# LukasHedegaard/continual-skeletons

Hardware: AMD Instinct MI355X
Metric: clips/sec (ST-GCN clip forward, NTU-60 shape; CoST-GCN online step reported under costgcn_online) (higher is better)
Workload: dtype f32

## Files before the change

### continual-skeletons_amd/csrc/gcn.hip

```cpp
#include <type_traits>

#include "mfma_core.h"
#include "gcn_params.h"


template <int MT, int NJ>
__global__ __launch_bounds__(NTHREADS, 2) void gcn_stage_kernel(const GcnParams p) {
    constexpr int NT = 16384 / MT;
    constexpr int WM = MT / 64;
    constexpr int TPC = NTHREADS / NT;
    constexpr int KPT = KC / TPC;
    extern __shared__ __attribute__((aligned(16))) float smem[];
    const int V = p.V, R = p.R, EW = p.ell_w;
    float *Wl = smem;
    float *Xa = Wl + R * KC * MT;
    float *Bx = Xa + R * KC * NT;
    float *Lv = Bx + KC * p.ldb;
    int *Ls = reinterpret_cast<int *>(Lv + 3 * V * EW * (p.adj_per_frame ? p.lds_frames : 1));

    const int tid = threadIdx.x, lane = tid & 63, wave = __builtin_amdgcn_readfirstlane(tid >> 6);
    const int wm = wave % WM, wn = wave / WM;
    const int l31 = lane & 31, kh = lane >> 5;
    const unsigned wid = xcd_contiguous_id(blockIdx.x, gridDim.x);
    const int m0 = (int)(wid % p.mtiles) * MT, q0 = (int)((wid / p.mtiles) % p.qtiles) * NT;
// ... 135 lines not shown
    } else {
#pragma unroll
        for (int mi = 0; mi < 2; ++mi)
#pragma unroll
            for (int g = 0; g < 16; ++g) bb[mi][g] = p.bias[rbase + mi * 32 + 4 * kh + (g & 3) + 8 * (g >> 2)];
#pragma unroll
        for (int ni = 0; ni < 2; ++ni) {
            const int qc = min(q0 + wn * 64 + ni * 32 + l31, Q - 1);
#pragma unroll
            for (int mi = 0; mi < 2; ++mi)
#pragma unroll
                for (int g = 0; g < 16; ++g) {
                    const int co = rbase + mi * 32 + 4 * kh + (g & 3) + 8 * (g >> 2);
                    rv[ni][mi][g] = ident ? seg_base[(int64_t)min(co, p.Cout - 1) * p.x_chan_stride + qc] : 0.f;
                }
        }
    }
#pragma unroll
    for (int mi = 0; mi < 2; ++mi)
#pragma unroll
        for (int g = 0; g < 16; ++g) {
            const float v0 = relu_nan(acc[mi][0][g] + bb[mi][g] + rv[0][mi][g]);
            const float v1 = relu_nan(acc[mi][1][g] + bb[mi][g] + rv[1][mi][g]);
            const auto sw = __builtin_amdgcn_permlane32_swap(__float_as_uint(v0), __float_as_uint(v1), false, false);
            acc[mi][0][g] = __uint_as_float(sw[0]);
            acc[mi][1][g] = __uint_as_float(sw[1]);
        }
    const int qb = q0 + wn * 64 + lane;
    const bool qv = qb < Q;
    if (full) {
        if (qv) {
            const unsigned qo = 4u * (unsigned)qb;
#pragma unroll
            for (int mi = 0; mi < 2; ++mi)
#pragma unroll
                for (int g = 0; g < 16; ++g) {
                    float *orow = oseg + (int64_t)(rbase + mi * 32 + (g & 3) + 8 * (g >> 2)) * p.y_chan_stride;
                    st_lane(orow, qo, acc[mi][0][g]);
                    st_lane(orow + 4 * p.y_chan_stride, qo, acc[mi][1][g]);
                }
        }
    } else {
#pragma unroll
        for (int mi = 0; mi < 2; ++mi)
#pragma unroll
            for (int g = 0; g < 16; ++g) {
                const int row0 = rbase + mi * 32 + (g & 3) + 8 * (g >> 2);
                if (qv && row0 < p.Cout) oseg[(int64_t)row0 * p.y_chan_stride + qb] = acc[mi][0][g];
                if (qv && row0 + 4 < p.Cout) oseg[(int64_t)(row0 + 4) * p.y_chan_stride + qb] = acc[mi][1][g];
            }
    }
}

template <int MT, bool CONVRES, int KCG_, bool PLAIN = false, bool SPLIT = false>
__global__ __launch_bounds__(NTHREADS, 3) void gcn_stage_sparse2_kernel(const GcnParams p) {
    constexpr int NT = 16384 / MT;
    constexpr int WM = MT / 64;
    constexpr int R = PLAIN ? 1 : (CONVRES ? 4 : 3);
    constexpr int M4 = MT / 4;
    constexpr int WB = (R * KCG_ * M4 + NTHREADS - 1) / NTHREADS;
    constexpr int RPW = KCG_ / (NTHREADS / 64);
    constexpr int NJ = MT == 128 ? 3 : 5;
    constexpr int NS = KCG_ / 2;
    constexpr int NH = NS / 2;
    static_assert(KCG_ % 8 == 0, "a chunk is a whole number of rows per wave");
    extern __shared__ __attribute__((aligned(16))) float smem[];
    const int V = p.V;
    const int wsz = R * KCG_ * MT, bsz = KCG_ * p.ldb, bufsz = wsz + bsz;

    const int tid = threadIdx.x, lane = tid & 63, wave = __builtin_amdgcn_readfirstlane(tid >> 6);
    const int wm = wave % WM, wn = wave / WM;
    const int l31 = lane & 31, kh = lane >> 5;
    const unsigned wid = xcd_contiguous_id(blockIdx.x, gridDim.x);
    const int m0 = (int)(wid % p.mtiles) * MT, q0 = (int)((wid / p.mtiles) % p.qtiles) * NT;
    const int segks = (int)(wid / (p.mtiles * p.qtiles));
    const int seg = SPLIT ? segks / p.ksplit : segks, ks = SPLIT ? segks % p.ksplit : 0;
    const int cb = SPLIT ? ks * p.cper : 0;
    const int Q = p.frames * V;
    const int qend = min(q0 + NT, Q);
    const int ta = div_magic(q0, p.vmagic), tb = div_magic(qend - 1, p.vmagic);
    const int span = (tb - ta + 1) * V;
    int eoff[2][6];
    float eval[2][6];
    int ioff[2];
#pragma unroll
    for (int ni = 0; ni < 2; ++ni) {
        const int q = min(q0 + wn * 64 + ni * 32 + l31, Q - 1);
        const int t = div_magic(q, p.vmagic);
        const int w = q - t * V, fb = (t - ta) * V;
        ioff[ni] = fb + w;
#pragma unroll
        for (int e = 0; e < 6; ++e) {
            const int r = e < 2 ? e : 2, k = e < 2 ? 0 : e - 2;
            const bool have = !PLAIN && k < p.ell_cnt[r];
            const int idx = PLAIN ? 0 : (r * V + w) * p.ell_w + min(k, p.ell_w - 1);
            eoff[ni][e] = fb + (have ? p.ell_src[idx] : 0);
            eval[ni][e] = have ? p.ell_val[idx] : 0.f;
        }
    }

    f32x16 acc[2][2];
#pragma unroll
    for (int a = 0; a < 2; ++a)
#pragma unroll
        for (int b = 0; b < 2; ++b)
#pragma unroll
            for (int g = 0; g < 16; ++g) acc[a][b][g] = 0.f;

    const float *seg_base = p.x + (int64_t)seg * p.x_seg_stride;
    const float *wbase = p.w + m0 + (size_t)cb * p.Mpad;
    f32x4 wv[WB];
    unsigned wgo[WB], wlo[WB];
#pragma unroll
    for (int u = 0; u < WB; ++u) {
        const int e = min(u * NTHREADS + tid, R * KCG_ * M4 - 1);
        const int row = e / M4, m4 = e % M4;
        wgo[u] = (unsigned)(((row / KCG_) * p.CinPad + (row % KCG_)) * p.Mpad + m4 * 4);
        wlo[u] = (unsigned)(e * 4);
    }
    constexpr int NJ4 = (NJ + 3) / 4;
    float bv[RPW][NJ];
    f32x4 bv4[RPW][NJ4];
    unsigned bgo[NJ], blo[NJ];
#pragma unroll
    for (int u = 0; u < NJ; ++u) {
        const int j = min(u * 64 + lane, span - 1);
        bgo[u] = (unsigned)(ta * V + j);
        blo[u] = (unsigned)j;
    }
    const int nvec = (span + 3) / 4;
    const bool vec = ta * V + 4 * nvec <= Q && p.Cin >= KCG_;
    unsigned bgo4[NJ4], blo4[NJ4];
#pragma unroll
    for (int u = 0; u < NJ4; ++u) {
        const int i = min(u * 64 + lane, nvec - 1);
        bgo4[u] = (unsigned)(ta * V + 4 * i);
        blo4[u] = (unsigned)(4 * i);
    }
    auto issue_one = [&](auto vtag, int i, int c0) {
        constexpr bool VEC = decltype(vtag)::value;
        constexpr int NX = VEC ? NJ4 : NJ;
        if (i < WB) {
            wv[i] = *reinterpret_cast<const f32x4 *>(wbase + (size_t)c0 * p.Mpad + wgo[i]);
        } else {
            const int rr = (i - WB) / NX, u = (i - WB) % NX;
            const int c = min(cb + c0 + wave + rr * (NTHREADS / 64), p.Cin - 1);
            const float *row = seg_base + (int64_t)c * p.x_chan_stride;
            if (VEC) bv4[rr][u] = *reinterpret_cast<const f32x4u *>(row + bgo4[u]);
            else bv[rr][u] = row[bgo[u]];
        }
    };
    auto commit = [&](auto vtag, float *buf) {
        constexpr bool VEC = decltype(vtag)::value;
        float *Wl = buf, *Bx = buf + wsz;
#pragma unroll
        for (int u = 0; u < WB; ++u) *reinterpret_cast<f32x4 *>(Wl + wlo[u]) = wv[u];
#pragma unroll
        for (int rr = 0; rr < RPW; ++rr) {
            float *dst = Bx + (wave + rr * (NTHREADS / 64)) * p.ldb;
            if (VEC) {
#pragma unroll
                for (int u = 0; u < NJ4; ++u) *reinterpret_cast<f32x4 *>(dst + blo4[u]) = bv4[rr][u];
            } else {
#pragma unroll
                for (int u = 0; u < NJ; ++u) dst[blo[u]] = bv[rr][u];
            }
        }
    };
    const int offA = wm * 64 + l31;
    auto mfma_step = [&](const float *buf, int s) {
        const float *Wl = buf, *Bx = buf + wsz;
        const int kk = 2 * s + kh;
        const float *bx = Bx + kk * p.ldb;
        float b[R][2];
#pragma unroll
        for (int ni = 0; ni < 2; ++ni) {
            if constexpr (PLAIN) {
                b[0][ni] = bx[ioff[ni]];
            } else {
                const float x0 = bx[eoff[ni][0]];
                b[0][ni] = eval[ni][0] * x0;
                b[1][ni] = eval[ni][1] * bx[eoff[ni][1]];
                float s2 = eval[ni][2] * bx[eoff[ni][2]];
                s2 = fmaf(eval[ni][3], bx[eoff[ni][3]], s2);
                s2 = fmaf(eval[ni][4], bx[eoff[ni][4]], s2);
                s2 = fmaf(eval[ni][5], bx[eoff[ni][5]], s2);
                b[2][ni] = s2;
                if (CONVRES) b[R - 1][ni] = bx[ioff[ni]];
            }
        }
#pragma unroll
        for (int r = 0; r < R; ++r) {
            const float *wr = Wl + (r * KCG_ + kk) * MT + offA;
            const float a0 = wr[0], a1 = wr[32];
            acc[0][0] = __builtin_amdgcn_mfma_f32_32x32x2f32(a0, b[r][0], acc[0][0], 0, 0, 0);
            acc[0][1] = __builtin_amdgcn_mfma_f32_32x32x2f32(a0, b[r][1], acc[0][1], 0, 0, 0);
            acc[1][0] = __builtin_amdgcn_mfma_f32_32x32x2f32(a1, b[r][0], acc[1][0], 0, 0, 0);
            acc[1][1] = __builtin_amdgcn_mfma_f32_32x32x2f32(a1, b[r][1], acc[1][1], 0, 0, 0);
        }
    };

    const int nchunks = (SPLIT ? min(p.CinPad - cb, p.cper) : p.CinPad) / KCG_;
    auto k_loop = [&](auto vtag) {
        constexpr int NLX = WB + RPW * (decltype(vtag)::value ? NJ4 : NJ);
#pragma unroll
        for (int i = 0; i < NLX; ++i) issue_one(vtag, i, 0);
        commit(vtag, smem);
        if (nchunks > 1) {
#pragma unroll
            for (int i = 0; i < NLX; ++i) issue_one(vtag, i, KCG_);
        }
        __syncthreads();
        for (int c = 0; c + 1 < nchunks; ++c) {
            float *cur = smem + (c & 1) * bufsz, *oth = smem + ((c & 1) ^ 1) * bufsz;
            commit(vtag, oth);
            const int cnext = min(c + 2, nchunks - 1) * KCG_;
            __builtin_amdgcn_s_setprio(1);
#pragma unroll
            for (int s = 0; s < NS; ++s) {
                if (s < NH) {
#pragma unroll
                    for (int i = s * NLX / NH; i < (s + 1) * NLX / NH; ++i) issue_one(vtag, i, cnext);
                    __builtin_amdgcn_sched_barrier(0);
                }
                mfma_step(cur, s);
            }
            __builtin_amdgcn_s_setprio(0);
            __syncthreads();
        }
    };
    if (vec) k_loop(std::true_type{});
    else k_loop(std::false_type{});
    const float *last = smem + ((nchunks - 1) & 1) * bufsz;
    const int rbase = m0 + wm * 64;
    const bool full = p.fast_epi && m0 + MT <= p.Cout;
    const unsigned kh4 = 4u * (unsigned)kh;
    float *oseg = SPLIT ? p.part + (int64_t)(seg * p.ksplit + ks) * p.Cout * p.y_chan_stride : p.y + (int64_t)seg * p.y_seg_stride;
    const int qb = q0 + wn * 64 + lane;
    const bool qv = qb < Q;
    float bb[2][16], rv[2][2][16];
    auto load_half = [&](int mi) {
        if (SPLIT) {
#pragma unroll
            for (int g = 0; g < 16; ++g) bb[mi][g] = rv[0][mi][g] = rv[1][mi][g] = 0.f;
        } else if (full) {
#pragma unroll
            for (int g = 0; g < 16; ++g) bb[mi][g] = ld_lane(p.bias + (rbase + mi * 32 + (g & 3) + 8 * (g >> 2)), kh4 * 4u);
#pragma unroll
            for (int ni = 0; ni < 2; ++ni) {
                const unsigned lo = 4u * (kh4 * (unsigned)p.x_chan_stride + (unsigned)min(q0 + wn * 64 + ni * 32 + l31, Q - 1));
#pragma unroll
                for (int g = 0; g < 16; ++g) {
                    const float *rrow = seg_base + (int64_t)(rbase + mi * 32 + (g & 3) + 8 * (g >> 2)) * p.x_chan_stride;
                    rv[ni][mi][g] = (CONVRES || PLAIN) ? 0.f : ld_lane(rrow, lo);
                }
            }
        } else {
#pragma unroll
            for (int g = 0; g < 16; ++g) bb[mi][g] = p.bias[rbase + mi * 32 + 4 * kh + (g & 3) + 8 * (g >> 2)];
#pragma unroll
            for (int ni = 0; ni < 2; ++ni) {
                const int qc = min(q0 + wn * 64 + ni * 32 + l31, Q - 1);
#pragma unroll
                for (int g = 0; g < 16; ++g) {
                    const int co = rbase + mi * 32 + 4 * kh + (g & 3) + 8 * (g >> 2);
                    rv[ni][mi][g] = (CONVRES || PLAIN) ? 0.f : seg_base[(int64_t)min(co, p.Cout - 1) * p.x_chan_stride + qc];
                }
            }
        }
    };
    auto finish_half = [&](int mi) {
#pragma unroll
        for (int g = 0; g < 16; ++g) {
            float v0 = acc[mi][0][g] + bb[mi][g] + rv[0][mi][g];
            float v1 = acc[mi][1][g] + bb[mi][g] + rv[1][mi][g];
            if (!PLAIN && !SPLIT) { v0 = relu_nan(v0); v1 = relu_nan(v1); }
            const auto sw = __builtin_amdgcn_permlane32_swap(__float_as_uint(v0), __float_as_uint(v1), false, false);
            acc[mi][0][g] = __uint_as_float(sw[0]);
            acc[mi][1][g] = __uint_as_float(sw[1]);
        }
        if (full) {
            if (qv) {
                const unsigned qo = 4u * (unsigned)qb;
#pragma unroll
                for (int g = 0; g < 16; ++g) {
                    float *orow = oseg + (int64_t)(rbase + mi * 32 + (g & 3) + 8 * (g >> 2)) * p.y_chan_stride;
                    st_lane(orow, qo, acc[mi][0][g]);
                    st_lane(orow + 4 * p.y_chan_stride, qo, acc[mi][1][g]);
                }
            }
        } else {
#pragma unroll
            for (int g = 0; g < 16; ++g) {
                const int row0 = rbase + mi * 32 + (g & 3) + 8 * (g >> 2);
                if (qv && row0 < p.Cout) oseg[(int64_t)row0 * p.y_chan_stride + qb] = acc[mi][0][g];
                if (qv && row0 + 4 < p.Cout) oseg[(int64_t)(row0 + 4) * p.y_chan_stride + qb] = acc[mi][1][g];
            }
        }
    };
#pragma unroll
    for (int s = 0; s < NS; ++s) mfma_step(last, s);
    load_half(0);
    finish_half(0);
    load_half(1);
    finish_half(1);
}

template <int MT, bool CONVRES, int KC2, int OCC>
__global__ __launch_bounds__(NTHREADS, OCC) void gcn_stage_dense_kernel(const GcnParams p) {
    constexpr int NT = 16384 / MT;
    constexpr int WM = MT / 64;
    constexpr int R = CONVRES ? 4 : 3;
    constexpr int M4 = MT / 4;
    constexpr int WB = R * KC2 * M4 / NTHREADS;
    constexpr int WBU = (R * KC2 * M4 + NTHREADS - 1) / NTHREADS;
    extern __shared__ __attribute__((aligned(16))) float smem[];
    const int V = p.V, FT = p.lds_frames, ldbx = p.ldb;
    float *Wl = smem;
    float *Xa = Wl + R * KC2 * MT;
    float *Bx = Xa + 3 * KC2 * NT;
    float *Ladj = Bx + KC2 * ldbx;

    const int tid = threadIdx.x, lane = tid & 63, wave = __builtin_amdgcn_readfirstlane(tid >> 6);
    const int wm = wave % WM, wn = wave / WM;
    const int l31 = lane & 31, kh = lane >> 5;
    const unsigned wid = xcd_contiguous_id(blockIdx.x, gridDim.x);
    const int m0 = (int)(wid % p.mtiles) * MT, qt = (int)((wid / p.mtiles) % p.qtiles);
    const int seg = (int)(wid / (p.mtiles * p.qtiles));
    const int Q = p.frames * V;
    const int ta = qt * FT, q0 = ta * V;
    const int fcnt = min(FT, p.frames - ta);
    const int ncol = fcnt * V;
    (void)WB;

    {
        const float *gv = p.ell_val + (int64_t)seg * p.adj_seg_stride;
        for (int e = tid; e < 3 * V * V; e += NTHREADS) Ladj[e] = gv[e];
    }
    f32x16 acc[2][2];
#pragma unroll
    for (int a = 0; a < 2; ++a)
#pragma unroll
        for (int b = 0; b < 2; ++b)
#pragma unroll
            for (int g = 0; g < 16; ++g) acc[a][b][g] = 0.f;

    const float *seg_base = p.x + (int64_t)seg * p.x_seg_stride;
    const float *wbase = p.w + m0;
    f32x4 wv[WBU];
    constexpr int XV = 2;
    const int nvec_row = (ncol + 3) / 4;
    const int xrow = tid / 32, xv0 = tid % 32;
    f32x4 xv[XV][2];
    auto issue = [&](int c0) {
#pragma unroll
        for (int u = 0; u < WBU; ++u) {
            const int e = min(u * NTHREADS + tid, R * KC2 * M4 - 1);
            const int row = e / M4, m4 = e % M4;
// ... 116 lines not shown
#pragma unroll
            for (int g = 0; g < 16; ++g) bb[g] = p.bias[rbase + mi * 32 + 4 * kh + (g & 3) + 8 * (g >> 2)];
#pragma unroll
            for (int ni = 0; ni < 2; ++ni) {
                const int qc = min(q0 + wn * 64 + ni * 32 + l31, Q - 1);
#pragma unroll
                for (int g = 0; g < 16; ++g) {
                    const int co = rbase + mi * 32 + 4 * kh + (g & 3) + 8 * (g >> 2);
                    rv[ni][g] = ident ? seg_base[(int64_t)min(co, p.Cout - 1) * p.x_chan_stride + qc] : 0.f;
                }
            }
        }
#pragma unroll
        for (int g = 0; g < 16; ++g) {
            const float v0 = relu_nan(acc[mi][0][g] + bb[g] + rv[0][g]);
            const float v1 = relu_nan(acc[mi][1][g] + bb[g] + rv[1][g]);
            const auto sw = __builtin_amdgcn_permlane32_swap(__float_as_uint(v0), __float_as_uint(v1), false, false);
            acc[mi][0][g] = __uint_as_float(sw[0]);
            acc[mi][1][g] = __uint_as_float(sw[1]);
        }
        if (full) {
            if (qv) {
                const unsigned qo = 4u * (unsigned)qb;
#pragma unroll
                for (int g = 0; g < 16; ++g) {
                    float *orow = oseg + (int64_t)(rbase + mi * 32 + (g & 3) + 8 * (g >> 2)) * p.y_chan_stride;
                    st_lane(orow, qo, acc[mi][0][g]);
                    st_lane(orow + 4 * p.y_chan_stride, qo, acc[mi][1][g]);
                }
            }
        } else {
#pragma unroll
            for (int g = 0; g < 16; ++g) {
                const int row0 = rbase + mi * 32 + (g & 3) + 8 * (g >> 2);
                if (qv && row0 < p.Cout) oseg[(int64_t)row0 * p.y_chan_stride + qb] = acc[mi][0][g];
                if (qv && row0 + 4 < p.Cout) oseg[(int64_t)(row0 + 4) * p.y_chan_stride + qb] = acc[mi][1][g];
            }
        }
    }
}

__global__ __launch_bounds__(256) void gcn_reduce_kernel(const GcnParams p) {
    const int Q = p.frames * p.V;
    const int64_t i = (int64_t)blockIdx.x * 256 + threadIdx.x;
    if (i >= (int64_t)p.Cout * Q) return;
    const int co = (int)(i / Q), q = (int)(i - (int64_t)co * Q), seg = blockIdx.y;
    float s = 0.f;
    for (int ks = 0; ks < p.ksplit; ++ks) s += p.part[((int64_t)(seg * p.ksplit + ks) * p.Cout + co) * p.y_chan_stride + q];
    s += p.bias[co];
    if (p.res_mode == CSK_RES_IDENTITY) s += p.x[(int64_t)seg * p.x_seg_stride + (int64_t)co * p.x_chan_stride + q];
    p.y[(int64_t)seg * p.y_seg_stride + (int64_t)co * p.y_chan_stride + q] = relu_nan(s);
}

static int gcn_stage_setup(const float *x, float *y, const float *w, const float *bias, const int32_t *ell_src, const float *ell_val,
                           const int32_t *ell_cnt, int ell_w, int64_t adj_seg_stride, int adj_per_frame, int n_seg, int c_in, int c_out,
                           int frames, int V, int64_t x_seg_stride, int64_t x_chan_stride, int64_t y_seg_stride, int64_t y_chan_stride,
                           int res_mode, int ksplit, float *partial, GcnParams *out, size_t *lds_out, bool *sparse_out) {
    if (n_seg <= 0 || c_in <= 0 || c_out <= 0 || frames <= 0 || V < 2 || V > 64) CSK_FAIL("gcn_stage: bad dims");
    if (ell_w < 1 || ell_w > V) CSK_FAIL("gcn_stage: ell_w must be in [1, V]");
    if (res_mode != CSK_RES_IDENTITY && res_mode != CSK_RES_CONV) CSK_FAIL("gcn_stage: res_mode must be identity or conv");
    if (res_mode == CSK_RES_IDENTITY && c_in != c_out) CSK_FAIL("gcn_stage: identity residual needs c_in == c_out");
    for (int i = 0; i < 3; ++i)
        if (ell_cnt[i] < 0 || ell_cnt[i] > ell_w) CSK_FAIL("gcn_stage: ell_cnt[%d] out of range", i);
    GcnParams &p = *out;
    p = gcn_params(x, y, w, bias, ell_src, ell_val, ell_cnt, ell_w, adj_seg_stride, c_in, c_out, frames, V, x_seg_stride,
                   x_chan_stride, y_seg_stride, y_chan_stride, res_mode, partial);
    p.dense = adj_seg_stride != 0 && ell_w == V && ell_cnt[0] == V && ell_cnt[1] == V && ell_cnt[2] == V;
    p.adj_per_frame = adj_per_frame != 0;
    if (p.adj_per_frame && !p.dense) CSK_FAIL("gcn_stage: per-frame adjacency must be dense (ell_w == V, ell_cnt == V)");
    const bool big = (p.Mpad % 128) == 0;
    const int MT = big ? 128 : 64, NT = 16384 / MT;
    const int max_dt = (NT + V - 2) / V;
    p.ldb = round_up((max_dt + 1) * V, 4);
    p.lds_frames = max_dt + 1;
    const size_t lds = (size_t)(p.R * KC * MT + p.R * KC * NT + KC * p.ldb + 3 * V * ell_w * (1 + (p.adj_per_frame ? p.lds_frames : 1))) * sizeof(float);
    if (lds > 160 * 1024) CSK_FAIL("gcn_stage: LDS tile %zu B exceeds 160 KiB", lds);
    const int Q = frames * V;
    if ((int64_t)frames * V >= (1 << 26)) CSK_FAIL("gcn_stage: frames*V too large for 32-bit position arithmetic");
    p.qtiles = (Q + NT - 1) / NT; p.mtiles = p.Mpad / MT;
    if ((int64_t)p.qtiles * p.mtiles * n_seg >= (1ll << 31)) CSK_FAIL("gcn_stage: grid too large");
    const bool sparse = adj_seg_stride == 0 && ell_cnt[0] <= 1 && ell_cnt[1] <= 1 && ell_cnt[2] <= 4 && p.ldb <= (big ? 192 : 320) &&
                        !csk_diag_flag("CSK_GCN_GENERAL");
    if (ksplit > 1 && !sparse) CSK_FAIL("gcn_stage_splitk: split-K is built for the skeleton-sparse kernel (shared adjacency, <= 1/1/4 non-zeros per column)");
    p.ksplit = split_ranges(p.CinPad, c_in, ksplit, 8, &p.cper);
    *lds_out = lds; *sparse_out = sparse;
    return 0;
}

static bool gcn16_candidate(const GcnParams &p, bool sparse) { return sparse && p.ksplit == 1; }

enum { ROUTE_UNIT = 1000000, ROUTE_SPARSE2 = 1, ROUTE_TILE16 = 2, ROUTE_DENSE2 = 3, ROUTE_DENSE128 = 4, ROUTE_GENERAL = 5 };
static int gcn_stage_route(const GcnParams &p, bool sparse, int n_seg) {
    const bool big = (p.Mpad % 128) == 0;
    const int MT = big ? 128 : 64, NT = 16384 / MT, V = p.V;
    if (gcn16_candidate(p, sparse)) {
        if (const int tile = csk_gcn16_tile(p, n_seg)) return ROUTE_TILE16 * ROUTE_UNIT + tile;
    }
    if (sparse) return ROUTE_SPARSE2 * ROUTE_UNIT + MT * 10 + (p.R == 4 ? 1 : 0);
    if (p.dense) {
        if (const int d2 = csk_gcn_dense2_route(p, n_seg)) return ROUTE_DENSE2 * ROUTE_UNIT + d2;
    }
    if (big && p.dense && !p.adj_per_frame && V >= 4 && V <= 32 && NT / V >= 1 && p.frames * (int64_t)V >= 4) {
        const int ft = NT / V;
        if ((int64_t)((p.frames + ft - 1) / ft) * p.mtiles * n_seg >= (1ll << 31)) CSK_FAIL("gcn_stage: grid too large");
        return ROUTE_DENSE128 * ROUTE_UNIT + (p.R == 4 ? 1 : 0);
    }
    const int nj = (p.ldb + 63) / 64;
    if (nj > (big ? 4 : 6)) CSK_FAIL("gcn_stage: activation tile of %d positions per channel exceeds the staged maximum", p.ldb);
    return ROUTE_GENERAL * ROUTE_UNIT + MT * 10 + (big ? (nj <= 3 ? 3 : 4) : (nj <= 5 ? 5 : 6));
}

static int gcn_stage_impl(const float *x, float *y, const float *w, const float *bias, const int32_t *ell_src,
                          const float *ell_val, const int32_t *ell_cnt, int ell_w, int64_t adj_seg_stride,
                          int adj_per_frame,
                          int n_seg, int c_in, int c_out, int frames, int V, int64_t x_seg_stride,
                          int64_t x_chan_stride, int64_t y_seg_stride, int64_t y_chan_stride, int res_mode,
                          int ksplit, float *partial, void *stream) {
    if (!x || !y || !w || !bias || !ell_src || !ell_val || !ell_cnt) CSK_FAIL("gcn_stage: null pointer");
    GcnParams p;
    size_t lds;
    bool sparse;
    if (const int rc = gcn_stage_setup(x, y, w, bias, ell_src, ell_val, ell_cnt, ell_w, adj_seg_stride, adj_per_frame, n_seg, c_in, c_out, frames,
                                       V, x_seg_stride, x_chan_stride, y_seg_stride, y_chan_stride, res_mode, ksplit, partial, &p, &lds, &sparse))
        return rc;
    const bool big = (p.Mpad % 128) == 0;
    const int MT = big ? 128 : 64, NT = 16384 / MT;
    const int Q = frames * V;
    dim3 grid(p.qtiles * p.mtiles * n_seg);
    const int route = gcn_stage_route(p, sparse, n_seg);
    if (route < 0) return route;
    const int family = route / ROUTE_UNIT;
    if (family == ROUTE_TILE16) return csk_launch_gcn16(p, n_seg, stream);
    if (family == ROUTE_SPARSE2) {
        const int R = p.R;
        size_t lds2;
        void (*k)(GcnParams);
        lds2 = 2 * (size_t)(R * 8 * MT + 8 * p.ldb) * sizeof(float);
        if (p.ksplit > 1) {
            if ((int64_t)p.qtiles * p.mtiles * n_seg * p.ksplit >= (1ll << 31)) CSK_FAIL("gcn_stage: grid too large");
            grid = dim3(p.qtiles * p.mtiles * n_seg * p.ksplit);
            k = big ? (R == 4 ? gcn_stage_sparse2_kernel<128, true, 8, false, true> : gcn_stage_sparse2_kernel<128, false, 8, false, true>)
                    : (R == 4 ? gcn_stage_sparse2_kernel<64, true, 8, false, true> : gcn_stage_sparse2_kernel<64, false, 8, false, true>);
        } else {
            k = big ? (R == 4 ? gcn_stage_sparse2_kernel<128, true, 8> : gcn_stage_sparse2_kernel<128, false, 8>)
                    : (R == 4 ? gcn_stage_sparse2_kernel<64, true, 8> : gcn_stage_sparse2_kernel<64, false, 8>);
        }
        const int e = csk_ensure_lds((const void *)k, lds2);
        if (e) return e;
        hipLaunchKernelGGL(k, grid, dim3(NTHREADS), lds2, (hipStream_t)stream, p);
        if (p.ksplit > 1) {
            if (const int e2 = (int)hipGetLastError()) return e2;
            const int64_t work = (int64_t)c_out * Q;
            hipLaunchKernelGGL(gcn_reduce_kernel, dim3((unsigned)((work + 255) / 256), n_seg), dim3(256), 0, (hipStream_t)stream, p);
        }
        return (int)hipGetLastError();
    }
    if (family == ROUTE_DENSE2) return csk_launch_gcn_dense2(p, n_seg, stream);
    if (family == ROUTE_DENSE128) {
        const int KC2 = 8;
        p.lds_frames = NT / V;
        int ldbx = round_up(p.lds_frames * V, 4);
        if ((ldbx / 4) % 2 == 0) ldbx += 4;
        p.ldb = ldbx;
        p.qtiles = (frames + p.lds_frames - 1) / p.lds_frames;
        const size_t ldsd = (size_t)(p.R * KC2 * MT + 3 * KC2 * NT + KC2 * ldbx + 3 * V * V) * sizeof(float);
        void (*kd)(GcnParams) = p.R == 4 ? gcn_stage_dense_kernel<128, true, 8, 3> : gcn_stage_dense_kernel<128, false, 8, 3>;
        if (const int e = csk_ensure_lds((const void *)kd, ldsd)) return e;
        hipLaunchKernelGGL(kd, dim3(p.qtiles * p.mtiles * n_seg), dim3(NTHREADS), ldsd, (hipStream_t)stream, p);
        return (int)hipGetLastError();
    }
    const int nj = route % 10;
    void (*kern)(GcnParams) = big ? (nj == 3 ? gcn_stage_kernel<128, 3> : gcn_stage_kernel<128, 4>)
                                  : (nj == 5 ? gcn_stage_kernel<64, 5> : gcn_stage_kernel<64, 6>);
    if (const int e = csk_ensure_lds((const void *)kern, lds)) return e;
    hipLaunchKernelGGL(kern, grid, dim3(NTHREADS), lds, (hipStream_t)stream, p);
    return (int)hipGetLastError();
}

extern "C" int csk_gcn_stage_f32(const float *x, float *y, const float *w, const float *bias, const int32_t *ell_src,
                                 const float *ell_val, const int32_t *ell_cnt, int ell_w, int64_t adj_seg_stride,
                                 int adj_per_frame,
                                 int n_seg, int c_in, int c_out, int frames, int V, int64_t x_seg_stride,
                                 int64_t x_chan_stride, int64_t y_seg_stride, int64_t y_chan_stride, int res_mode,
                                 void *stream) {
    return gcn_stage_impl(x, y, w, bias, ell_src, ell_val, ell_cnt, ell_w, adj_seg_stride, adj_per_frame, n_seg, c_in, c_out, frames,
                          V, x_seg_stride, x_chan_stride, y_seg_stride, y_chan_stride, res_mode, 1, nullptr, stream);
}

extern "C" int csk_gcn_stage_f32_tile(const float *x, const float *y, const int32_t *ell_cnt, int ell_w, int64_t adj_seg_stride,
                                      int adj_per_frame, int n_seg, int c_in, int c_out, int frames, int V, int64_t x_seg_stride,
                                      int64_t x_chan_stride, int64_t y_seg_stride, int64_t y_chan_stride, int res_mode) {
    if (!ell_cnt) CSK_FAIL("gcn_stage: null pointer");
    GcnParams p;
    size_t lds;
    bool sparse;
    if (const int rc = gcn_stage_setup(x, const_cast<float *>(y), nullptr, nullptr, nullptr, nullptr, ell_cnt, ell_w, adj_seg_stride, adj_per_frame,
                                       n_seg, c_in, c_out, frames, V, x_seg_stride, x_chan_stride, y_seg_stride, y_chan_stride, res_mode, 1,
                                       nullptr, &p, &lds, &sparse))
        return rc;
    return gcn16_candidate(p, sparse) ? csk_gcn16_tile(p, n_seg) : 0;
}

extern "C" int csk_gcn_stage_f32_route(const float *x, const float *y, const float *ell_val, const int32_t *ell_cnt, int ell_w,
                                       int64_t adj_seg_stride, int adj_per_frame, int n_seg, int c_in, int c_out, int frames, int V,
                                       int64_t x_seg_stride, int64_t x_chan_stride, int64_t y_seg_stride, int64_t y_chan_stride,
                                       int res_mode) {
    if (!ell_cnt) CSK_FAIL("gcn_stage: null pointer");
    GcnParams p;
    size_t lds;
    bool sparse;
    if (const int rc = gcn_stage_setup(x, const_cast<float *>(y), nullptr, nullptr, nullptr, ell_val, ell_cnt, ell_w, adj_seg_stride, adj_per_frame,
                                       n_seg, c_in, c_out, frames, V, x_seg_stride, x_chan_stride, y_seg_stride, y_chan_stride, res_mode, 1,
                                       nullptr, &p, &lds, &sparse))
        return rc;
    return gcn_stage_route(p, sparse, n_seg);
}

extern "C" int csk_gcn_stage_splitk_f32(const float *x, float *y, const float *w, const float *bias, const int32_t *ell_src,
                                        const float *ell_val, const int32_t *ell_cnt, int ell_w, int n_seg, int c_in, int c_out,
                                        int frames, int V, int64_t x_seg_stride, int64_t x_chan_stride, int64_t y_seg_stride,
                                        int64_t y_chan_stride, int res_mode, int ksplit, float *partial, void *stream) {
    if (ksplit < 1 || ksplit > 32 || (ksplit > 1 && !partial)) CSK_FAIL("gcn_stage_splitk: ksplit must be in [1, 32] and needs a partial-sum buffer");
    return gcn_stage_impl(x, y, w, bias, ell_src, ell_val, ell_cnt, ell_w, 0, 0, n_seg, c_in, c_out, frames, V, x_seg_stride,
                          x_chan_stride, y_seg_stride, y_chan_stride, res_mode, ksplit, partial, stream);
}


extern "C" int csk_conv1x1_f32(const float *x, float *y, const float *w, const float *bias, int n_seg, int c_in, int c_out,
                               int frames, int V, int64_t x_seg_stride, int64_t x_chan_stride, int64_t y_seg_stride,
                               int64_t y_chan_stride, void *stream) {
    if (!x || !y || !w || !bias) CSK_FAIL("conv1x1: null pointer");
    if (n_seg <= 0 || c_in <= 0 || c_out <= 0 || frames <= 0 || V < 2 || V > 64) CSK_FAIL("conv1x1: bad dims");
    if ((int64_t)frames * V >= (1 << 26)) CSK_FAIL("conv1x1: frames*V too large for 32-bit position arithmetic");
    const int32_t no_adjacency[3] = {0, 0, 0};
    GcnParams p = gcn_params(x, y, w, bias, nullptr, nullptr, no_adjacency, 1, 0, c_in, c_out, frames, V, x_seg_stride, x_chan_stride,
                             y_seg_stride, y_chan_stride, CSK_RES_NONE, nullptr);
    p.R = 1;
    const bool big = (p.Mpad % 128) == 0;
    const int MT = big ? 128 : 64, NT = 16384 / MT;
    const int max_dt = (NT + V - 2) / V;
    p.ldb = round_up((max_dt + 1) * V, 4);
    if (p.ldb > (big ? 192 : 320)) CSK_FAIL("conv1x1: activation tile of %d positions exceeds the staged maximum", p.ldb);
    const int Q = frames * V;
    p.qtiles = (Q + NT - 1) / NT; p.mtiles = p.Mpad / MT;
    if ((int64_t)p.qtiles * p.mtiles * n_seg >= (1ll << 31)) CSK_FAIL("conv1x1: grid too large");
    constexpr int KCP = 16;
    const size_t lds = 2 * (size_t)(KCP * MT + KCP * p.ldb) * sizeof(float);
    void (*k)(GcnParams) = big ? gcn_stage_sparse2_kernel<128, false, KCP, true> : gcn_stage_sparse2_kernel<64, false, KCP, true>;
    if (const int e = csk_ensure_lds((const void *)k, lds)) return e;
    hipLaunchKernelGGL(k, dim3(p.qtiles * p.mtiles * n_seg), dim3(NTHREADS), lds, (hipStream_t)stream, p);
    return (int)hipGetLastError();
}
```

### continual-skeletons_amd/native.py

```python
import ctypes as C
import os

import torch

_HERE = os.path.dirname(os.path.abspath(__file__))
LIB_PATH = os.path.join(_HERE, "libcskel_hip.so")
ABI_VERSION = 16

_p, _i, _l = C.c_void_p, C.c_int, C.c_int64
SIGNATURES = {
    "csk_abi_version": [],
    "csk_stream_overlap_probe": [C.c_void_p, C.c_void_p, C.c_int, C.POINTER(C.c_float)],
    "csk_gcn_stage_f32": [_p, _p, _p, _p, _p, _p, _p, _i, _l, _i, _i, _i, _i, _i, _i, _l, _l, _l, _l, _i, _p],
    "csk_gcn_stage_f32_tile": [_p, _p, _p, _i, _l, _i, _i, _i, _i, _i, _i, _l, _l, _l, _l, _i],
    "csk_gcn_stage_f32_route": [_p, _p, _p, _p, _i, _l, _i, _i, _i, _i, _i, _i, _l, _l, _l, _l, _i],
    "csk_gcn_stage_splitk_f32": [_p, _p, _p, _p, _p, _p, _p, _i, _i, _i, _i, _i, _i, _l, _l, _l, _l, _i, _i, _p, _p],
    "csk_tcn_stage_f32": [_p, _p, _p, _p, _p, _p, _i, _i, _i, _i, _i, _i, _i, _i, _i, _i, _i, _i, _i, _p],
    "csk_tcn_stage_wino_f32": [_p, _p, _p, _p, _p, _p, _i, _i, _i, _i, _i, _i, _i, _i, _i, _i, _i, _i, _i, _p, _p],
    "csk_tcn_stage_wino_ext_f32": [_p, _p, _p, _p, _p, _p, _i, _i, _i, _i, _i, _i, _i, _i, _i, _i, _i, _i, _i, _p, _p],
    "csk_tcn_stage_wino_valid_f32": [_p, _p, _p, _p, _p, _p, _i, _i, _i, _i, _i, _i, _i, _i, _i, _i, _i, _i, _i, _p, _p],
    "csk_tcn_stage_wino_valid_res_f32": [_p, _p, _p, _p, _p, _i, _i, _i, _i, _i, _i, _i, _i, _i, _i, _i, _i, _i, _p, _p],
    "csk_block_few_channels_f32": [_p, _p, _p, _p, _p, _p, _i, _p, _p, _p, _i, _i, _i, _i, _i, _i, _i, _p],
    "csk_tcn_stage_splitk_f32": [_p, _p, _p, _p, _p, _p, _i, _i, _i, _i, _i, _i, _i, _i, _i, _i, _i, _i, _i, _i, _p, _p],
    "csk_conv1x1_f32": [_p, _p, _p, _p, _i, _i, _i, _i, _i, _l, _l, _l, _l, _p],
    "csk_tcn_stage_bf16x3": [_p, _p, _p, _p, _p, _p, _i, _i, _i, _i, _i, _i, _i, _i, _i, _i, _i, _i, _i, _p],
    "csk_gcn_stage_bf16x3": [_p, _p, _p, _p, _p, _p, _p, _p, _i, _i, _i, _i, _i, _i, _i, _p],
    "csk_input_norm_f32": [_p, _p, _p, _p, _i, _i, _i, _i, _i, _l, _l, _p],
    "csk_pool_fc_f32": [_p, _p, _p, _p, _p, _i, _i, _i, _i, _i, _p],
    "csk_fc_f32": [_p, _p, _p, _p, _i, _i, _i, _p],
    "csk_pool_scaled_f32": [_p, _p, _i, _i, _i, _i, C.c_float, _p],
    "csk_agcn_attention_f32": [_p, _p, _p, _p, _i, _i, _i, _i, _l, _l, _i, _l, _p],
    "csk_agcn_embed_attention_f32": [_p, _p, _p, _p, _p, _p, _i, _i, _i, _i, _i, _i, _l, _l, _p],
    "csk_tcn_step_f32": [_p, _i, _i, _i, _i, _p, _p, _i, _i, _i, _p, _p, _p, _i, _i, _i, _i, _l, _i, _i, _i, _i, _i, _p, _p],
    "csk_tcn_step_f32_tile": [_i, _i, _i, _i, _i, _i, _i, _l, _i, _i, _i, _i],
    "csk_tcn_step_bf16x3": [_p, _i, _i, _i, _i, _p, _p, _i, _i, _i, _p, _p, _p, _i, _i, _i, _i, _l, _i, _i, _i, _i, _p],
    "csk_tcn_step_bf16x3_tile": [_i, _i, _l],
    "csk_co_stack_step_f32": [_i, _p, _i, _i, _l, _p],
    "csk_co_block_step_f32": [_p, _i, _i, _i, _p, _p, _p, _p, _p, _i, _i, _p, _i, _i, _p, _p, _i, _i, _p, _i, _i, _i, _i, _i, _l, _p],
    "csk_co_spatial_pool_f32": [_p, _p, _i, _i, _i, _l, _p],
    "csk_co_window_mean_f32": [_p, _p, _l, _i, _i, _i, _p],
    "csk_co_head_step_f32": [_p, _p, _p, _p, _p, _p, _i, _i, _i, _l, _i, _i, _i, _i, _i, _p],
    "csk_input_norm_frames_f32": [_p, _p, _i, _p, _p, _i, _i, _i, _i, _l, _p],
    "csk_derive_modality_f32": [_p, _p, _i, _p, _i, _i, _i, _i, _i, _p],
    "csk_derive_modality_frames_f32": [_p, _p, _i, _i, _p, _p, _p, _i, _i, _i, _i, _i, _p],
    "csk_prenorm_f32": [_p, _p, _i, _i, _i, _i, _i, _i, _i, _i, _p],
    "csk_prenorm_frames_f32": [_p, _p, _i, _p, _p, _i, _i, _i, _i, _i, _i, _i, _i, _p],

    "csk_fuse_rank_f32": [_p, _i, _i, _i, _i, _l, _l, _p, _p, _p, _p],
    "csk_co_plan_create": [_i, _p, _p, _i, _i, _i, _i, _i, _l, _p, _p, _i, _p, _p, _i, _i, _p, _p],
    "csk_co_plan_destroy": [_p],
    "csk_co_plan_update_weights": [_p, _i, _p, _p, _p, _p, _p],
    "csk_co_plan_set_fusion": [_p, _i],
    "csk_co_plan_set_delays": [_p, _i, _p],
    "csk_co_plan_cycle": [_p, C.POINTER(C.c_int64), _i, _p, _i, _p, _p, _p, _p, _p],
    "csk_co_scrub_streams_f32": [_p, _i, _p, _i, _i, _p],
    "csk_co_move_streams_f32": [_p, _i, _p, _l, _p, _i, _i, _i, _p],
    "csk_str_unit_f32": [_p, _p, _p, _l, _p, _p, _p, _p, _p, _p, _p, _i, _i, _i, _i, _i, _l, _l, _l, _l, _p],
}
RESTYPES = {"csk_co_plan_create": C.c_void_p, "csk_co_plan_destroy": None}


class CoLayer(C.Structure):
    _fields_ = [("c_in", C.c_int32), ("c_out", C.c_int32), ("stride", C.c_int32), ("res_kind", C.c_int32),
                ("gcn_res_mode", C.c_int32), ("ell_w", C.c_int32), ("ell_cnt", C.c_int32 * 3), ("tcn_ksplit", C.c_int32),
                ("y_slots", C.c_int32), ("out_slots", C.c_int32), ("partial_emits", C.c_int32), ("agcn_adj_frames", C.c_int32),
                ("gcn_ksplit", C.c_int32), ("gcn_partial_frames", C.c_int32),
                ("gcn_w", C.c_void_p), ("gcn_bias", C.c_void_p), ("ell_src", C.c_void_p), ("ell_val", C.c_void_p),
                ("tcn_w", C.c_void_p), ("tcn_w_res", C.c_void_p), ("tcn_bias", C.c_void_p),
# ... 73 lines not shown
```

### include/cskel.h

```cpp
#ifndef CSKEL_H
#define CSKEL_H

#include <stdint.h>

#ifdef __cplusplus
extern "C" {
#endif

#define CSK_ABI_VERSION 16
#define CSK_KC 8
#define CSK_CPAD 16
#define CSK_MT 64

#define CSK_RES_NONE 0
#define CSK_RES_IDENTITY 1
#define CSK_RES_CONV 2

int csk_abi_version(void);
const char *csk_last_error(void);

int csk_stream_overlap_probe(void *stream_a, void *stream_b, int spin_us, float *ratio);

int csk_gcn_stage_f32(const float *x, float *y, const float *w, const float *bias,
                      const int32_t *ell_src, const float *ell_val, const int32_t *ell_cnt,
                      int ell_w, int64_t adj_seg_stride, int adj_per_frame,
                      int n_seg, int c_in, int c_out, int frames, int V,
                      int64_t x_seg_stride, int64_t x_chan_stride,
                      int64_t y_seg_stride, int64_t y_chan_stride,
                      int res_mode, void *stream);

int csk_gcn_stage_f32_tile(const float *x, const float *y, const int32_t *ell_cnt, int ell_w, int64_t adj_seg_stride,
                           int adj_per_frame, int n_seg, int c_in, int c_out, int frames, int V,
                           int64_t x_seg_stride, int64_t x_chan_stride, int64_t y_seg_stride, int64_t y_chan_stride,
                           int res_mode);

int csk_gcn_stage_f32_route(const float *x, const float *y, const float *ell_val, const int32_t *ell_cnt, int ell_w,
                            int64_t adj_seg_stride, int adj_per_frame, int n_seg, int c_in, int c_out, int frames, int V,
                            int64_t x_seg_stride, int64_t x_chan_stride, int64_t y_seg_stride, int64_t y_chan_stride,
                            int res_mode);

int csk_gcn_stage_splitk_f32(const float *x, float *y, const float *w, const float *bias, const int32_t *ell_src,
                             const float *ell_val, const int32_t *ell_cnt, int ell_w, int n_seg, int c_in, int c_out,
                             int frames, int V, int64_t x_seg_stride, int64_t x_chan_stride, int64_t y_seg_stride,
                             int64_t y_chan_stride, int res_mode, int ksplit, float *partial, void *stream);

int csk_tcn_stage_f32(const float *y, const float *w, const float *x_res, const float *w_res,
                      const float *bias, float *out,
                      int n_seg, int c, int c_out, int t_in, int V, int k, int stride, int pad,
                      int res_mode, int c_res, int t_res, int res_off, int relu, void *stream);

int csk_tcn_stage_wino_f32(const float *y, const float *w, const float *x_res, const float *w_res,
                           const float *bias, float *out,
                           int n_seg, int c, int c_out, int t_in, int V, int k, int stride, int pad,
                           int res_mode, int c_res, int t_res, int res_off, int relu, const float *w_wino, void *stream);

int csk_tcn_stage_wino_ext_f32(const float *y, const float *w, const float *x_res, const float *w_res,
                               const float *bias, float *out,
                               int n_seg, int c, int c_out, int t_in, int V, int k, int stride, int pad,
                               int res_mode, int c_res, int t_res, int res_off, int relu, const float *w_wino_ext, void *stream);

int csk_tcn_stage_wino_valid_f32(const float *y, const float *w, const float *x_res, const float *w_res,
                                 const float *bias, float *out,
                                 int n_seg, int c, int c_out, int t_in, int V, int k, int stride, int pad,
                                 int res_mode, int c_res, int t_res, int res_off, int relu, const float *w_wino, void *stream);

int csk_tcn_stage_wino_valid_res_f32(const float *y, const float *x_res, const float *w_res, const float *bias, float *out,
                                     int n_seg, int c, int c_out, int t_in, int V, int k, int stride, int pad,
                                     int res_mode, int c_res, int t_res, int res_off, int relu, const float *w_wino, void *stream);

int csk_block_few_channels_f32(const float *x, const float *gcn_w, const float *gcn_bias, const int32_t *ell_src,
                               const float *ell_val, const int32_t *ell_cnt, int ell_w, const float *tcn_w,
                               const float *tcn_bias, float *out, int n_seg, int c_in, int c_mid, int c_out, int t_in,
                               int V, int pad, void *stream);

int csk_tcn_stage_splitk_f32(const float *y, const float *w, const float *x_res, const float *w_res,
                             const float *bias, float *out,
                             int n_seg, int c, int c_out, int t_in, int V, int k, int stride, int pad,
                             int res_mode, int c_res, int t_res, int res_off, int relu, int ksplit, float *partial,
                             void *stream);

int csk_conv1x1_f32(const float *x, float *y, const float *w, const float *bias, int n_seg, int c_in, int c_out,
                    int frames, int V, int64_t x_seg_stride, int64_t x_chan_stride, int64_t y_seg_stride,
                    int64_t y_chan_stride, void *stream);

int csk_tcn_stage_bf16x3(const float *y, const void *w_split, const float *x_res, const void *w_res_split,
                         const float *bias, float *out,
                         int n_seg, int c, int c_out, int t_in, int V, int k, int stride, int pad,
                         int res_mode, int c_res, int t_res, int res_off, int relu, void *stream);

int csk_gcn_stage_bf16x3(const float *x, float *y, const void *w_split, const void *w_res_split, const float *bias,
                         const int32_t *ell_src, const float *ell_val, const int32_t *ell_cnt, int ell_w,
                         int n_seg, int c_in, int c_out, int frames, int V, int res_mode, void *stream);
// ... 161 lines not shown
```

Measured before the change: 4336.

## Add tall 128x256 wave tile variant of sparse GCN kernel for 128->256 conv-residual stage

Adds an MI=4 variant of the sparse skeleton GCN kernel where each wave covers all 128 output rows of a 128-row workgroup tile, with a 256-column position tile. Each B operand built from the adjacency gather is now reused across four MFMA row blocks instead of two, which cuts the per-MFMA cost of the gather and LDS reads. The variant is routed only for conv-residual stages with c_in 128 and c_out 256. In exchange it uses more accumulator registers and drops occupancy to 2 workgroups, and the grid has fewer, larger tiles.

After: 4355, median of 6. Within noise of the previous version (+0.4%).

```diff
diff --git a/continual-skeletons_amd/csrc/gcn.hip b/continual-skeletons_amd/csrc/gcn.hip
--- a/continual-skeletons_amd/csrc/gcn.hip
+++ b/continual-skeletons_amd/csrc/gcn.hip
@@ -211,15 +211,16 @@
     }
 }
 
-template <int MT, bool CONVRES, int KCG_, bool PLAIN = false, bool SPLIT = false>
-__global__ __launch_bounds__(NTHREADS, 3) void gcn_stage_sparse2_kernel(const GcnParams p) {
-    constexpr int NT = 16384 / MT;
-    constexpr int WM = MT / 64;
+template <int MT, bool CONVRES, int KCG_, bool PLAIN = false, bool SPLIT = false, int MI = 2>
+__global__ __launch_bounds__(NTHREADS, MI == 4 ? 2 : 3) void gcn_stage_sparse2_kernel(const GcnParams p) {
+    static_assert(MI == 2 || (MI == 4 && MT == 128), "wave tile: 64 rows, or all 128 rows of a 128-row workgroup tile");
+    constexpr int WM = MT / (32 * MI);
+    constexpr int NT = 64 * (NTHREADS / 64) / WM;
     constexpr int R = PLAIN ? 1 : (CONVRES ? 4 : 3);
     constexpr int M4 = MT / 4;
     constexpr int WB = (R * KCG_ * M4 + NTHREADS - 1) / NTHREADS;
     constexpr int RPW = KCG_ / (NTHREADS / 64);
-    constexpr int NJ = MT == 128 ? 3 : 5;
+    constexpr int NJ = NT == 128 ? 3 : 5;
     constexpr int NS = KCG_ / 2;
     constexpr int NH = NS / 2;
     static_assert(KCG_ % 8 == 0, "a chunk is a whole number of rows per wave");
@@ -258,9 +259,9 @@
         }
     }
 
-    f32x16 acc[2][2];
-#pragma unroll
-    for (int a = 0; a < 2; ++a)
+    f32x16 acc[MI][2];
+#pragma unroll
+    for (int a = 0; a < MI; ++a)
 #pragma unroll
         for (int b = 0; b < 2; ++b)
 #pragma unroll
@@ -326,7 +327,7 @@
             }
         }
     };
-    const int offA = wm * 64 + l31;
+    const int offA = wm * 32 * MI + l31;
     auto mfma_step = [&](const float *buf, int s) {
         const float *Wl = buf, *Bx = buf + wsz;
         const int kk = 2 * s + kh;
@@ -356,6 +357,13 @@
             acc[0][1] = __builtin_amdgcn_mfma_f32_32x32x2f32(a0, b[r][1], acc[0][1], 0, 0, 0);
             acc[1][0] = __builtin_amdgcn_mfma_f32_32x32x2f32(a1, b[r][0], acc[1][0], 0, 0, 0);
             acc[1][1] = __builtin_amdgcn_mfma_f32_32x32x2f32(a1, b[r][1], acc[1][1], 0, 0, 0);
+            if constexpr (MI == 4) {
+                const float a2 = wr[64], a3 = wr[96];
+                acc[2][0] = __builtin_amdgcn_mfma_f32_32x32x2f32(a2, b[r][0], acc[2][0], 0, 0, 0);
+                acc[2][1] = __builtin_amdgcn_mfma_f32_32x32x2f32(a2, b[r][1], acc[2][1], 0, 0, 0);
+                acc[3][0] = __builtin_amdgcn_mfma_f32_32x32x2f32(a3, b[r][0], acc[3][0], 0, 0, 0);
+                acc[3][1] = __builtin_amdgcn_mfma_f32_32x32x2f32(a3, b[r][1], acc[3][1], 0, 0, 0);
+            }
         }
     };
 
@@ -391,13 +399,13 @@
     if (vec) k_loop(std::true_type{});
     else k_loop(std::false_type{});
     const float *last = smem + ((nchunks - 1) & 1) * bufsz;
-    const int rbase = m0 + wm * 64;
+    const int rbase = m0 + wm * 32 * MI;
     const bool full = p.fast_epi && m0 + MT <= p.Cout;
     const unsigned kh4 = 4u * (unsigned)kh;
     float *oseg = SPLIT ? p.part + (int64_t)(seg * p.ksplit + ks) * p.Cout * p.y_chan_stride : p.y + (int64_t)seg * p.y_seg_stride;
     const int qb = q0 + wn * 64 + lane;
     const bool qv = qb < Q;
-    float bb[2][16], rv[2][2][16];
+    float bb[MI][16], rv[2][MI][16];
     auto load_half = [&](int mi) {
         if (SPLIT) {
 #pragma unroll
@@ -463,6 +471,12 @@
     finish_half(0);
     load_half(1);
     finish_half(1);
+    if constexpr (MI == 4) {
+        load_half(2);
+        finish_half(2);
+        load_half(3);
+        finish_half(3);
+    }
 }
 
 template <int MT, bool CONVRES, int KC2, int OCC>
@@ -685,10 +699,22 @@
     p.y[(int64_t)seg * p.y_seg_stride + (int64_t)co * p.y_chan_stride + q] = relu_nan(s);
 }
 
+static bool gcn_tall_gate(int c_out, int V) {
+    return c_out > 0 && c_out % 128 == 0 && V >= 2 && round_up(((256 + V - 2) / V + 1) * V, 4) <= 320;
+}
+static bool gcn_tall_pick(int c_in, int c_out, int V, int res_mode, int force) {
+    if (!gcn_tall_gate(c_out, V)) return false;
+    if (force == 2 || force == 3) return force == 3;
+    return res_mode == CSK_RES_CONV && c_in == 128 && c_out == 256;
+}
+extern "C" int csk_gcn_stage_f32_tall(int c_in, int c_out, int V, int res_mode) {
+    return gcn_tall_pick(c_in, c_out, V, res_mode, csk_diag_int("CSK_GCN_GENERAL")) ? 1 : 0;
+}
+
 static int gcn_stage_setup(const float *x, float *y, const float *w, const float *bias, const int32_t *ell_src, const float *ell_val,
                            const int32_t *ell_cnt, int ell_w, int64_t adj_seg_stride, int adj_per_frame, int n_seg, int c_in, int c_out,
                            int frames, int V, int64_t x_seg_stride, int64_t x_chan_stride, int64_t y_seg_stride, int64_t y_chan_stride,
-                           int res_mode, int ksplit, float *partial, GcnParams *out, size_t *lds_out, bool *sparse_out) {
+                           int res_mode, int ksplit, float *partial, GcnParams *out, size_t *lds_out, bool *sparse_out, bool *tall_out) {
     if (n_seg <= 0 || c_in <= 0 || c_out <= 0 || frames <= 0 || V < 2 || V > 64) CSK_FAIL("gcn_stage: bad dims");
     if (ell_w < 1 || ell_w > V) CSK_FAIL("gcn_stage: ell_w must be in [1, V]");
     if (res_mode != CSK_RES_IDENTITY && res_mode != CSK_RES_CONV) CSK_FAIL("gcn_stage: res_mode must be identity or conv");
@@ -702,7 +728,11 @@
     p.adj_per_frame = adj_per_frame != 0;
     if (p.adj_per_frame && !p.dense) CSK_FAIL("gcn_stage: per-frame adjacency must be dense (ell_w == V, ell_cnt == V)");
     const bool big = (p.Mpad % 128) == 0;
-    const int MT = big ? 128 : 64, NT = 16384 / MT;
+    const int force = csk_diag_int("CSK_GCN_GENERAL");
+    const bool skel = adj_seg_stride == 0 && ell_cnt[0] <= 1 && ell_cnt[1] <= 1 && ell_cnt[2] <= 4 &&
+                      !(csk_diag_flag("CSK_GCN_GENERAL") && force < 2);
+    const bool tall = skel && ksplit <= 1 && gcn_tall_pick(c_in, c_out, V, res_mode, force);
+    const int MT = big ? 128 : 64, NT = tall ? 256 : 16384 / MT;
     const int max_dt = (NT + V - 2) / V;
     p.ldb = round_up((max_dt + 1) * V, 4);
     p.lds_frames = max_dt + 1;
@@ -712,24 +742,23 @@
     if ((int64_t)frames * V >= (1 << 26)) CSK_FAIL("gcn_stage: frames*V too large for 32-bit position arithmetic");
     p.qtiles = (Q + NT - 1) / NT; p.mtiles = p.Mpad / MT;
     if ((int64_t)p.qtiles * p.mtiles * n_seg >= (1ll << 31)) CSK_FAIL("gcn_stage: grid too large");
-    const bool sparse = adj_seg_stride == 0 && ell_cnt[0] <= 1 && ell_cnt[1] <= 1 && ell_cnt[2] <= 4 && p.ldb <= (big ? 192 : 320) &&
-                        !csk_diag_flag("CSK_GCN_GENERAL");
+    const bool sparse = skel && p.ldb <= (NT == 128 ? 192 : 320);
     if (ksplit > 1 && !sparse) CSK_FAIL("gcn_stage_splitk: split-K is built for the skeleton-sparse kernel (shared adjacency, <= 1/1/4 non-zeros per column)");
     p.ksplit = split_ranges(p.CinPad, c_in, ksplit, 8, &p.cper);
-    *lds_out = lds; *sparse_out = sparse;
+    *lds_out = lds; *sparse_out = sparse; *tall_out = tall;
     return 0;
 }
 
 static bool gcn16_candidate(const GcnParams &p, bool sparse) { return sparse && p.ksplit == 1; }
 
 enum { ROUTE_UNIT = 1000000, ROUTE_SPARSE2 = 1, ROUTE_TILE16 = 2, ROUTE_DENSE2 = 3, ROUTE_DENSE128 = 4, ROUTE_GENERAL = 5 };
-static int gcn_stage_route(const GcnParams &p, bool sparse, int n_seg) {
+static int gcn_stage_route(const GcnParams &p, bool sparse, bool tall, int n_seg) {
     const bool big = (p.Mpad % 128) == 0;
     const int MT = big ? 128 : 64, NT = 16384 / MT, V = p.V;
-    if (gcn16_candidate(p, sparse)) {
+    if (gcn16_candidate(p, sparse) && csk_diag_int("CSK_GCN_GENERAL") < 2) {
         if (const int tile = csk_gcn16_tile(p, n_seg)) return ROUTE_TILE16 * ROUTE_UNIT + tile;
     }
-    if (sparse) return ROUTE_SPARSE2 * ROUTE_UNIT + MT * 10 + (p.R == 4 ? 1 : 0);
+    if (sparse) return ROUTE_SPARSE2 * ROUTE_UNIT + (tall ? 10000 : 0) + MT * 10 + (p.R == 4 ? 1 : 0);
     if (p.dense) {
         if (const int d2 = csk_gcn_dense2_route(p, n_seg)) return ROUTE_DENSE2 * ROUTE_UNIT + d2;
     }
@@ -752,15 +781,15 @@
     if (!x || !y || !w || !bias || !ell_src || !ell_val || !ell_cnt) CSK_FAIL("gcn_stage: null pointer");
     GcnParams p;
     size_t lds;
-    bool sparse;
+    bool sparse, tall;
     if (const int rc = gcn_stage_setup(x, y, w, bias, ell_src, ell_val, ell_cnt, ell_w, adj_seg_stride, adj_per_frame, n_seg, c_in, c_out, frames,
-                                       V, x_seg_stride, x_chan_stride, y_seg_stride, y_chan_stride, res_mode, ksplit, partial, &p, &lds, &sparse))
+                                       V, x_seg_stride, x_chan_stride, y_seg_stride, y_chan_stride, res_mode, ksplit, partial, &p, &lds, &sparse, &tall))
         return rc;
     const bool big = (p.Mpad % 128) == 0;
     const int MT = big ? 128 : 64, NT = 16384 / MT;
     const int Q = frames * V;
     dim3 grid(p.qtiles * p.mtiles * n_seg);
-    const int route = gcn_stage_route(p, sparse, n_seg);
+    const int route = gcn_stage_route(p, sparse, tall, n_seg);
     if (route < 0) return route;
     const int family = route / ROUTE_UNIT;
     if (family == ROUTE_TILE16) return csk_launch_gcn16(p, n_seg, stream);
@@ -774,6 +803,8 @@
             grid = dim3(p.qtiles * p.mtiles * n_seg * p.ksplit);
             k = big ? (R == 4 ? gcn_stage_sparse2_kernel<128, true, 8, false, true> : gcn_stage_sparse2_kernel<128, false, 8, false, true>)
                     : (R == 4 ? gcn_stage_sparse2_kernel<64, true, 8, false, true> : gcn_stage_sparse2_kernel<64, false, 8, false, true>);
+        } else if (route % ROUTE_UNIT >= 10000) {
+            k = R == 4 ? gcn_stage_sparse2_kernel<128, true, 8, false, false, 4> : gcn_stage_sparse2_kernel<128, false, 8, false, false, 4>;
         } else {
             k = big ? (R == 4 ? gcn_stage_sparse2_kernel<128, true, 8> : gcn_stage_sparse2_kernel<128, false, 8>)
                     : (R == 4 ? gcn_stage_sparse2_kernel<64, true, 8> : gcn_stage_sparse2_kernel<64, false, 8>);
@@ -826,10 +857,10 @@
     if (!ell_cnt) CSK_FAIL("gcn_stage: null pointer");
     GcnParams p;
     size_t lds;
-    bool sparse;
+    bool sparse, tall;
     if (const int rc = gcn_stage_setup(x, const_cast<float *>(y), nullptr, nullptr, nullptr, nullptr, ell_cnt, ell_w, adj_seg_stride, adj_per_frame,
                                        n_seg, c_in, c_out, frames, V, x_seg_stride, x_chan_stride, y_seg_stride, y_chan_stride, res_mode, 1,
-                                       nullptr, &p, &lds, &sparse))
+                                       nullptr, &p, &lds, &sparse, &tall))
         return rc;
     return gcn16_candidate(p, sparse) ? csk_gcn16_tile(p, n_seg) : 0;
 }
@@ -841,12 +872,12 @@
     if (!ell_cnt) CSK_FAIL("gcn_stage: null pointer");
     GcnParams p;
     size_t lds;
-    bool sparse;
+    bool sparse, tall;
     if (const int rc = gcn_stage_setup(x, const_cast<float *>(y), nullptr, nullptr, nullptr, ell_val, ell_cnt, ell_w, adj_seg_stride, adj_per_frame,
                                        n_seg, c_in, c_out, frames, V, x_seg_stride, x_chan_stride, y_seg_stride, y_chan_stride, res_mode, 1,
-                                       nullptr, &p, &lds, &sparse))
+                                       nullptr, &p, &lds, &sparse, &tall))
         return rc;
-    return gcn_stage_route(p, sparse, n_seg);
+    return gcn_stage_route(p, sparse, tall, n_seg);
 }
 
 extern "C" int csk_gcn_stage_splitk_f32(const float *x, float *y, const float *w, const float *bias, const int32_t *ell_src,
diff --git a/continual-skeletons_amd/native.py b/continual-skeletons_amd/native.py
--- a/continual-skeletons_amd/native.py
+++ b/continual-skeletons_amd/native.py
@@ -14,6 +14,7 @@
     "csk_gcn_stage_f32": [_p, _p, _p, _p, _p, _p, _p, _i, _l, _i, _i, _i, _i, _i, _i, _l, _l, _l, _l, _i, _p],
     "csk_gcn_stage_f32_tile": [_p, _p, _p, _i, _l, _i, _i, _i, _i, _i, _i, _l, _l, _l, _l, _i],
     "csk_gcn_stage_f32_route": [_p, _p, _p, _p, _i, _l, _i, _i, _i, _i, _i, _i, _l, _l, _l, _l, _i],
+    "csk_gcn_stage_f32_tall": [_i, _i, _i, _i],
     "csk_gcn_stage_splitk_f32": [_p, _p, _p, _p, _p, _p, _p, _i, _i, _i, _i, _i, _i, _l, _l, _l, _l, _i, _i, _p, _p],
     "csk_tcn_stage_f32": [_p, _p, _p, _p, _p, _p, _i, _i, _i, _i, _i, _i, _i, _i, _i, _i, _i, _i, _i, _p],
     "csk_tcn_stage_wino_f32": [_p, _p, _p, _p, _p, _p, _i, _i, _i, _i, _i, _i, _i, _i, _i, _i, _i, _i, _i, _p, _p],
diff --git a/include/cskel.h b/include/cskel.h
--- a/include/cskel.h
+++ b/include/cskel.h
@@ -38,6 +38,8 @@
                             int64_t adj_seg_stride, int adj_per_frame, int n_seg, int c_in, int c_out, int frames, int V,
                             int64_t x_seg_stride, int64_t x_chan_stride, int64_t y_seg_stride, int64_t y_chan_stride,
                             int res_mode);
+
+int csk_gcn_stage_f32_tall(int c_in, int c_out, int V, int res_mode);
 
 int csk_gcn_stage_splitk_f32(const float *x, float *y, const float *w, const float *bias, const int32_t *ell_src,
                              const float *ell_val, const int32_t *ell_cnt, int ell_w, int n_seg, int c_in, int c_out,
```
